# big-nacho/patolette

Hardware: AMD Instinct MI355X
Metric: Mpixels/sec quantized (256-color ICtCp + KMeans) at 1 GPU; palette ΔE vs ref (higher is better)
Workload: dtype f64

## Files before the change

include/patolette_amd.h:

```cpp
#ifndef PATOLETTE_AMD_H
#define PATOLETTE_AMD_H

#include <stddef.h>
#include <stdint.h>

#include "patolette.h"

#ifdef __cplusplus
extern "C" {
#endif

int  patolette_amd_device_count(void);
int  patolette_amd_set_device(int ordinal);
const char *patolette_amd_last_error(void);
void *patolette_amd_malloc(size_t bytes);
void patolette_amd_free(void *dptr);
int  patolette_amd_memcpy_h2d(void *dst, const void *src, size_t bytes);
int  patolette_amd_memcpy_d2h(void *dst, const void *src, size_t bytes);
int  patolette_amd_synchronize(void);
void patolette_amd_release_workspace(void);
int  patolette_amd_fill_image(double *d_planar, size_t n, uint64_t seed);
int  patolette_amd_fill_weights(double *d_weights, size_t n, uint64_t seed);

void patolette_amd_device(size_t width, size_t height, const double *d_data, const double *d_weights,
// ... 169 lines not shown
    PAMD_SRGB_TO_CIELUV = 1,
    PAMD_ICTCP_TO_REC2020 = 2,
    PAMD_CIELUV_TO_REC2020 = 3,
    PAMD_SRGB_TO_REC2020 = 4,
    PAMD_REC2020_TO_SRGB = 5,
    PAMD_CIELUV_TO_ICTCP = 6
};
int patolette_amd_convert(int which, double *planar, size_t n);

int patolette_amd_quantize_clusters(const double *colors, const double *weights, size_t n, size_t K,
                                    double *centers, size_t *n_clusters);

int patolette_amd_kmeans_refine(const double *colors, const double *weights, size_t n,
                                double *centers_io, size_t k, int niter, size_t max_samples);
int patolette_amd_debug_km_route(void);

int patolette_amd_nn_map(const double *colors, size_t n, const double *palette, size_t k, size_t *map);
int patolette_amd_debug_nn_route(int route);
int patolette_amd_debug_nn_map_elem(const double *colors, size_t n, const double *palette, size_t k, int map_elem_bytes, int misalign,
                                    void *map);

int patolette_amd_dither(const double *colors, size_t width, size_t height, const double *palette,
                         size_t k, size_t *map);

void patolette_amd_dither_config(int segments, int warm);
void patolette_amd_dither_layout(int lanes);
int patolette_amd_debug_dither_solo_cap(int cap);
int patolette_amd_debug_dither_stall_passes(int n);
int patolette_amd_dither_layout_in_use(size_t width, size_t height, size_t palette_rows);
void patolette_amd_debug_dither_locate(size_t width, size_t height, unsigned long long t, unsigned long long *d, unsigned long long *c);
// ... 54 lines not shown
```

patolette_amd/_native.py:

```python
import ctypes as C
import os

HERE = os.path.dirname(os.path.abspath(__file__))
LIB_PATH = os.path.join(HERE, "lib", "libpatolette_amd.so")

dp = C.POINTER(C.c_double)
zp = C.POINTER(C.c_size_t)


class QuantizationOptions(C.Structure):
    _fields_ = [("dither", C.c_bool), ("palette_only", C.c_bool), ("color_space", C.c_int),
                ("kmeans_niter", C.c_int), ("kmeans_max_samples", C.c_size_t), ("verbose", C.c_bool)]


class Stats(C.Structure):
    _fields_ = [(n, C.c_double) for n in ("ms_total", "ms_upload", "ms_convert", "ms_gq", "ms_lq",
                                          "ms_kmeans", "ms_map", "ms_download", "ms_saliency")] + \
               [(n, C.c_size_t) for n in ("n_base_clusters", "n_clusters", "split_evals", "split_px",
                                          "lq_rounds", "kmeans_samples", "dither_segments", "dither_repairs",
                                          "dither_rounds", "dither_through", "dither_jumps", "dither_solo")]

    def as_dict(self):
        return {n: getattr(self, n) for n, _ in self._fields_}

# ... 99 lines not shown
    "patolette_amd_hist_palette": (None, [C.c_void_p, C.c_int, C.c_size_t, C.POINTER(QuantizationOptions), dp, C.c_void_p,
                                          C.POINTER(C.c_int)]),
    "patolette_amd_batch": (None, [C.c_size_t, C.c_size_t, C.c_size_t, C.POINTER(dp), C.POINTER(dp), C.c_double, C.c_size_t,
                                   C.POINTER(QuantizationOptions), C.POINTER(dp), C.POINTER(zp), C.POINTER(C.c_int)]),
    "patolette_amd_batch_rows": (None, [C.c_size_t, C.c_size_t, C.c_size_t, C.POINTER(dp), C.POINTER(dp), C.c_double, C.c_size_t,
                                        C.POINTER(QuantizationOptions), C.POINTER(dp), C.POINTER(zp), C.POINTER(C.c_int)]),
    "patolette_amd_batch_u8": (None, [C.c_size_t, C.c_size_t, C.c_size_t, C.POINTER(C.c_void_p), C.c_int, C.POINTER(dp), C.c_double, C.c_size_t,
                                      C.POINTER(QuantizationOptions), C.POINTER(dp), C.POINTER(C.c_void_p), C.POINTER(C.c_void_p), C.c_int,
                                      C.POINTER(C.c_void_p), C.POINTER(C.c_int)]),
    "patolette_amd_pow": (C.c_int, [dp, C.c_double, dp, C.c_size_t]),
    "patolette_amd_convert": (C.c_int, [C.c_int, dp, C.c_size_t]),
    "patolette_amd_quantize_clusters": (C.c_int, [dp, dp, C.c_size_t, C.c_size_t, dp, zp]),
    "patolette_amd_kmeans_refine": (C.c_int, [dp, dp, C.c_size_t, dp, C.c_size_t, C.c_int, C.c_size_t]),
    "patolette_amd_nn_map": (C.c_int, [dp, C.c_size_t, dp, C.c_size_t, zp]),
    "patolette_amd_debug_km_route": (C.c_int, []),
    "patolette_amd_debug_nn_route": (C.c_int, [C.c_int]),
    "patolette_amd_debug_nn_map_elem": (C.c_int, [dp, C.c_size_t, dp, C.c_size_t, C.c_int, C.c_int, C.c_void_p]),
    "patolette_amd_set_global_quantiser": (C.c_int, [C.c_int]),
    "patolette_amd_dither": (C.c_int, [dp, C.c_size_t, C.c_size_t, dp, C.c_size_t, zp]),
    "patolette_amd_dither_config": (None, [C.c_int, C.c_int]),
    "patolette_amd_dither_layout": (None, [C.c_int]),
    "patolette_amd_debug_dither_solo_cap": (C.c_int, [C.c_int]),
    "patolette_amd_debug_dither_stall_passes": (C.c_int, [C.c_int]),
    "patolette_amd_dither_layout_in_use": (C.c_int, [C.c_size_t, C.c_size_t, C.c_size_t]),
    "patolette_amd_debug_dither_locate": (None, [C.c_size_t, C.c_size_t, C.c_ulonglong, C.POINTER(C.c_ulonglong),
                                                 C.POINTER(C.c_ulonglong)]),
    "patolette_amd_last_stats": (None, [C.POINTER(Stats)]),
    "patolette_amd_last_map_palette": (C.c_size_t, [dp, C.c_size_t]),
    "patolette_amd_last_split_trace": (C.c_size_t, [C.POINTER(SplitTrace), C.POINTER(SplitRecord), C.c_size_t]),
    "patolette_amd_last_cluster_centers": (C.c_size_t, [dp, C.c_size_t]),
# ... 79 lines not shown
```

patolette_amd/csrc/kmeans.h:

```cpp
#pragma once

#include "common.h"
#include "devutil.h"

namespace pamd {

constexpr int kKMeansMaxK = 4096;

struct KmSamples { float *x, *y, *z, *w; };

struct KMeansWork {
    DevBuf<float> sx, sy, sz, sw;
    DevBuf<int> assign;
    DevBuf<float4> sorted;
    DevBuf<unsigned int> table, rowtot, ticket;
    DevBuf<unsigned int> flags;
    DevBuf<unsigned int> rowbase;
    DevBuf<float> hs;
    DevBuf<float> cent, hassign;
    DevBuf<float4> c4;
    DevBuf<int> perm;
    DevBuf<struct DevMT> mt;
    bool mt_seeded = false;
    DevBuf<unsigned char> lut, grid, clist;
    DevBuf<unsigned int> mid;
    DevBuf<unsigned int> bkeys;
    DevBuf<unsigned long long> fsum;
    int route = 0;
    void reserve(size_t nx, int k);
};

enum KmRoute {
    KM_ROUTE_LIST = 1 << 0, KM_ROUTE_SCAN = 1 << 1, KM_ROUTE_BIGK = 1 << 2, KM_ROUTE_G32 = 1 << 3, KM_ROUTE_G64 = 1 << 4,
    KM_ROUTE_MID = 1 << 5, KM_ROUTE_SCATTER_INT = 1 << 6, KM_ROUTE_SCATTER_BYTE = 1 << 7, KM_ROUTE_SCATTER_PAIR = 1 << 8,
    KM_ROUTE_SCATTER_LDS = 1 << 9, KM_ROUTE_COOP = 1 << 10, KM_ROUTE_SUMS = 1 << 11
};

void kmeans_gather(const double *d_planar, size_t N, bool weighted, const int *d_perm, size_t nx, KMeansWork &w, hipStream_t s);
void kmeans_gather_slice(const double *d_planar, size_t n_local, bool weighted, const int *d_perm, size_t nx, size_t begin,
                         KMeansWork &w, hipStream_t s);
struct KmSums { double bound_x, bound_w; };
void kmeans_iterate(KMeansWork &w, size_t nx, int k, bool weighted, int niter, hipStream_t s, size_t expect_longest = 0,
                    const KmSums *sums = nullptr);

}
```

patolette_amd/csrc/kmeans.hip:

```cpp
#include "kmeans.h"

namespace pamd {

typedef __attribute__((address_space(1))) const void gvoid_t;
typedef __attribute__((address_space(3))) void lvoid_t;

template <bool W>
__global__ __launch_bounds__(256) void k_km_gather(const double *__restrict__ planar, size_t N, const int *__restrict__ perm,
                                                   size_t nx, KmSamples s) {
    const size_t stride = (size_t)gridDim.x * blockDim.x;
    for (size_t i = (size_t)blockIdx.x * blockDim.x + threadIdx.x; i < nx; i += stride) {
        size_t p = perm ? (size_t)perm[i] : i;
        s.x[i] = (float)planar[p]; s.y[i] = (float)planar[N + p]; s.z[i] = (float)planar[2 * N + p];
        if constexpr (W) s.w[i] = (float)planar[3 * N + p];
    }
}

template <bool W>
__global__ __launch_bounds__(256) void k_km_gather_slice(const double *__restrict__ planar, size_t n_local, const int *__restrict__ perm,
                                                         size_t nx, size_t begin, KmSamples s) {
    const size_t stride = (size_t)gridDim.x * blockDim.x;
    for (size_t i = (size_t)blockIdx.x * blockDim.x + threadIdx.x; i < nx; i += stride) {
        const size_t g = perm ? (size_t)perm[i] : i;
        const bool mine = g >= begin && g - begin < n_local;
// ... 1799 lines not shown
        __shared__ float s_hs[kKMeansMaxK];
        km_split_clusters_wave(cent, hassign, k, nx, mt, s_mt, s_hs, (int)threadIdx.x);
        __threadfence();
    }
    __syncthreads();
    for (int j = threadIdx.x; j < k; j += 256) km_store_c4(c4, k, j, cent[3 * j], cent[3 * j + 1], cent[3 * j + 2]);
}

static int chunk_len_for(size_t nx) {
    size_t c = ceil_div(nx, 4096);
    c = ceil_div(c, 64) * 64;
    if (c < 64) c = 64;
    return (int)c;
}

void KMeansWork::reserve(size_t nx, int k) {
    sx.reserve(nx); sy.reserve(nx); sz.reserve(nx); sw.reserve(nx);
    assign.reserve(nx); sorted.reserve(nx);
    const int nchunks = (int)ceil_div(nx, (size_t)chunk_len_for(nx));
    table.reserve(std::max((size_t)k * (size_t)(nchunks > 0 ? nchunks : 1),
                           (ceil_div(nx, (size_t)1024) * 257 + 1) / 2 + 1));
    rowtot.reserve(k);
    if (k > kKMeansMaxK) { rowbase.reserve(k); hs.reserve(k); }
    cent.reserve(3 * (size_t)k); hassign.reserve(k); c4.reserve(2 * (size_t)k + 2);
    perm.reserve(nx);
    if (!mt.p) { mt.reserve(1); mt_seeded = false; }
    if (!ticket.p) { ticket.reserve(1); HIP_CHECK(hipMemset(ticket.p, 0, sizeof(unsigned int))); }
    flags.reserve(2 + 256);
}

void kmeans_gather(const double *d_planar, size_t N, bool weighted, const int *d_perm, size_t nx, KMeansWork &w, hipStream_t s) {
    KmSamples ks{w.sx.p, w.sy.p, w.sz.p, w.sw.p};
    size_t g = ceil_div(nx, 256);
    if (g > 4096) g = 4096;
    if (g < 1) g = 1;
    KTIME("k_km_gather", s, (weighted ? 48.0 : 36.0) * nx);
// ... 2 lines not shown
    HIP_CHECK(hipGetLastError());
}

void kmeans_gather_slice(const double *d_planar, size_t n_local, bool weighted, const int *d_perm, size_t nx, size_t begin,
                         KMeansWork &w, hipStream_t s) {
    KmSamples ks{w.sx.p, w.sy.p, w.sz.p, w.sw.p};
    size_t g = ceil_div(nx, 256);
    if (g > 4096) g = 4096;
    if (g < 1) g = 1;
    KTIME("k_km_gather", s, (weighted ? 48.0 : 36.0) * nx);
    if (weighted) hipLaunchKernelGGL(k_km_gather_slice<true>, (int)g, 256, 0, s, d_planar, n_local, d_perm, nx, begin, ks);
    else hipLaunchKernelGGL(k_km_gather_slice<false>, (int)g, 256, 0, s, d_planar, n_local, d_perm, nx, begin, ks);
    HIP_CHECK(hipGetLastError());
}

void kmeans_iterate(KMeansWork &w, size_t nx, int k, bool weighted, int niter, hipStream_t s, size_t expect_longest, const KmSums *sums) {
    KmSamples ks{w.sx.p, w.sy.p, w.sz.p, w.sw.p};
    KmFix fix{};
    int ablocks = 1;
    if (sums && k > kKMeansMaxK) sums = nullptr;
    if (sums) {
        int ex = 0, ew = 0, P = 1;
        (void)frexp(std::max(sums->bound_x, 1e-300) * (weighted ? std::max(sums->bound_w, 1e-300) : 1.0), &ex);
        (void)frexp(std::max(sums->bound_w, 1e-300), &ew);
        while (((size_t)1 << P) < nx) P++;
        P = std::max(P + 1, 12);
        fix.quantum_x = ldexp(1.0, ex + P - 62); fix.magic_x = ldexp(1.5, 52 + ex + P - 62);
        fix.quantum_w = ldexp(1.0, ew + P - 62); fix.magic_w = ldexp(1.5, 52 + ew + P - 62);
        w.fsum.reserve(4 * (size_t)k);
        HIP_CHECK(hipMemsetAsync(w.fsum.p, 0, 4 * (size_t)k * sizeof(unsigned long long), s));
        ablocks = (int)std::min<size_t>(std::max<size_t>(ceil_div(nx, (size_t)4096), 1), 2048);
// ... 29 lines not shown
    const bool bigk = k > kKMeansMaxK;
    const size_t lds_cnt = bigk ? 0 : (size_t)8 * k * sizeof(unsigned int);
    const size_t lds_sct = (size_t)5 * k * sizeof(unsigned int);
    const size_t lds_sct_pair = (size_t)9 * k * sizeof(unsigned int) + (size_t)4 * (k + 64) * sizeof(float4);
    static PerDeviceOnce attr;
    attr.once([&] {
        HIP_CHECK(hipFuncSetAttribute((const void *)k_km_assign_count<false>, hipFuncAttributeMaxDynamicSharedMemorySize, 8 * kKMeansMaxK * 4));
        HIP_CHECK(hipFuncSetAttribute((const void *)k_km_scatter<true, int>, hipFuncAttributeMaxDynamicSharedMemorySize, 5 * kKMeansMaxK * 4));
        HIP_CHECK(hipFuncSetAttribute((const void *)k_km_scatter<false, int>, hipFuncAttributeMaxDynamicSharedMemorySize, 5 * kKMeansMaxK * 4));
        HIP_CHECK(hipFuncSetAttribute((const void *)k_km_scatter<true, unsigned char>, hipFuncAttributeMaxDynamicSharedMemorySize, 5 * kKMeansMaxK * 4));
        HIP_CHECK(hipFuncSetAttribute((const void *)k_km_scatter<false, unsigned char>, hipFuncAttributeMaxDynamicSharedMemorySize, 5 * kKMeansMaxK * 4));
        HIP_CHECK(hipFuncSetAttribute((const void *)k_km_update<true, false>, hipFuncAttributeMaxDynamicSharedMemorySize, 4 * 4096 * 4));
        HIP_CHECK(hipFuncSetAttribute((const void *)k_km_update<false, false>, hipFuncAttributeMaxDynamicSharedMemorySize, 4 * 4096 * 4));
    });
    if (!w.mt_seeded) { hipLaunchKernelGGL(k_km_mt_seed, 1, 1, 0, s, w.mt.p); w.mt_seeded = true; }
    { KTIME("k_km_prep", s, 28.0 * k); hipLaunchKernelGGL(k_km_prep, (std::max(k, kKmFlagWords) + 255) / 256, 256, 0, s, w.cent.p, k, w.c4.p, w.flags.p); }
    const size_t lut_min = getenv("PAMD_KM_LUT_MIN") ? (size_t)atoll(getenv("PAMD_KM_LUT_MIN")) : ((size_t)1 << 21);
    const bool use_lut = nx >= lut_min && k >= 16 && k <= 256;
    const size_t g64_min = getenv("PAMD_KM_G64_MIN") ? (size_t)atoll(getenv("PAMD_KM_G64_MIN")) : ((size_t)1 << 23);
    const int G = nx >= g64_min ? 64 : 32;
    if (use_lut) {
        static PerDeviceOnce attr2;
        attr2.once([&] {
            HIP_CHECK(hipFuncSetAttribute((const void *)k_km_assign_lut, hipFuncAttributeMaxDynamicSharedMemorySize, 8 * kKMeansMaxK * 4));
        });
        w.lut.reserve((size_t)G * G * G * 16); w.bkeys.reserve(kKmSlots * 6); w.grid.reserve(64 + sizeof(double));
        w.clist.reserve((size_t)(G * G * G / 64) * (2 + kKmCoarseMax));
        hipLaunchKernelGGL(k_km_bounds_init, 1, 256, 0, s, w.bkeys.p);
        { KTIME("k_km_bounds", s, 12.0 * nx); hipLaunchKernelGGL(k_km_bounds, (int)std::min<size_t>(ceil_div(nx, 256), 2048), 256, 0, s, ks, nx, w.bkeys.p); }
        hipLaunchKernelGGL(k_km_bounds_fold, 1, 64, 0, s, w.bkeys.p, (KmGridDev *)w.grid.p);
    }
    constexpr size_t direct_max = (size_t)1 << 19;
    const size_t list_longest = getenv("PAMD_KM_LIST_LONGEST") ? (size_t)atoll(getenv("PAMD_KM_LIST_LONGEST")) : (size_t)16384;
    const bool use_direct = !sums && !use_lut && k <= 256 && nx <= direct_max && nx < ((size_t)1 << 32) && expect_longest < list_longest;
    if (use_direct) {
        HIP_CHECK(hipMemsetAsync(w.assign.p, 0, nx, s));
        static PerDeviceOnce attr4;
        attr4.once([&] {
            HIP_CHECK(hipFuncSetAttribute((const void *)k_km_update_lists<true>, hipFuncAttributeMaxDynamicSharedMemorySize, kKmDirectCap * 20));
            HIP_CHECK(hipFuncSetAttribute((const void *)k_km_update_lists<false>, hipFuncAttributeMaxDynamicSharedMemorySize, kKmDirectCap * 20));
        });
    }
    const bool use_mid = use_lut && G == 64 && k % 8 == 0;
    if (use_mid) w.mid.reserve(32 * 32 * 32);
    const unsigned long long long_min = getenv("PAMD_KM_LONG_MIN") ? (unsigned long long)atoll(getenv("PAMD_KM_LONG_MIN")) : 8192ULL;
    int route = 0;
    for (int it = 0; it < niter; it++) {
        if (use_direct) {
            route |= KM_ROUTE_LIST;
            unsigned short *offs = (unsigned short *)w.table.p;
            const int sblocks = (int)ceil_div(nx, (size_t)kKmSortBlock);
// ... 129 lines not shown
```

patolette_amd/csrc/map.h:

```cpp
#pragma once

#include "common.h"

namespace pamd {

struct NNWork {
    DevBuf<unsigned char> lut;
    DevBuf<unsigned long long> keys;
    DevBuf<unsigned char> clist;
    DevBuf<unsigned int> mid;
    DevBuf<double> dtab;
    DevBuf<unsigned int> dside;
    PinBuf<unsigned int> hrep;
    DevBuf<double> dsort;
    DevBuf<unsigned int> dpos;
    size_t order_w = 0, order_h = 0; int order_dev = -1;
    DevBuf<unsigned int> dmpos;
    DevBuf<unsigned int> dmcnt;
    DevBuf<unsigned char> dsmap;
    DevBuf<unsigned char> dflag;
    size_t dither_segments = 0, dither_repairs = 0, dither_rounds = 0;
    size_t dither_through = 0;
    size_t dither_jumps = 0;
    size_t dither_solo = 0;
// ... 1 lines not shown
    hipEvent_t ev_fork = nullptr, ev_join = nullptr, ev_join2 = nullptr;
    int side_dev = -1;
    NNWork() = default;
    NNWork(const NNWork &) = delete;
    NNWork &operator=(const NNWork &) = delete;
    ~NNWork() {
        if (ev_fork) (void)hipEventDestroy(ev_fork);
        if (ev_join) (void)hipEventDestroy(ev_join);
        if (ev_join2) (void)hipEventDestroy(ev_join2);
        if (side_stream) (void)hipStreamDestroy(side_stream);
        if (side_stream2) (void)hipStreamDestroy(side_stream2);
    }
};
void launch_nn_map(const double *d_colors, size_t plane_stride, size_t n, const double *d_pal, int k,
                   void *d_out, int elem_bytes, const double *lo, const double *hi, NNWork &w, hipStream_t s);
int nn_debug_route(int route);
bool nn_map_u8_applies(size_t n, int k);
void launch_nn_map_u8(const unsigned char *d_px, int channels, size_t n, const double *d_pal, int k, void *d_out, int elem_bytes, NNWork &w, hipStream_t s);
bool dither_lane_layout(size_t width, size_t height, int k);
void launch_dither(const double *d_img, size_t plane_stride, int which, size_t width, size_t height, const double *d_pal, const double *h_pal, int k,
                   void *d_out, int elem_bytes, NNWork &w, hipStream_t s, int layout = -1);

constexpr size_t kDitherFramesMaxPixels = (size_t)1 << 31;
bool dither_frames_lane_layout(size_t frames, size_t width, size_t height, int k);
void launch_dither_frames(const double *d_img, size_t plane_stride, int which, size_t frames, size_t width, size_t height, const double *d_pal,
                          const double *h_pal, int k, void *d_out, int elem_bytes, NNWork &w, hipStream_t s, int layout = -1);

bool launch_dither_u8(const unsigned char *d_px, int channels, size_t frames, size_t width, size_t height, const double *d_pal, const double *h_pal,
                      int k, void *d_out, int elem_bytes, NNWork &w, hipStream_t s);

// ... 12 lines not shown
```

patolette_amd/csrc/map.hip:

```cpp
#include "map.h"
#include "compact.h"
#include "dither_slots.h"

#include <algorithm>
#include <atomic>
#include <cmath>
#include <mutex>
#include <type_traits>

#define PAMD_POW_TABLES_IN_LDS
#include "color_device.h"
#include "devutil.h"

namespace pamd {

template <typename OutT>
__global__ __launch_bounds__(256) void k_nn_map(const double *__restrict__ c, size_t N, size_t n, const double *__restrict__ pal, int k,
                                                OutT *__restrict__ out) {
    const double *palx = pal, *paly = pal + k, *palz = pal + 2 * k;
    const size_t stride = (size_t)gridDim.x * blockDim.x;
    for (size_t i = (size_t)blockIdx.x * blockDim.x + threadIdx.x; i < n; i += stride) {
        const double x = c[i], y = c[N + i], z = c[2 * N + i];
        double bd = INFINITY; int best = 0;
        for (int j = 0; j < k; j++) {
// ... 791 lines not shown
    attr_mid.once([&] { HIP_CHECK(hipFuncSetAttribute((const void *)(k_nn_map_mid<OutT, P, WAVES, NNSrcU8>), hipFuncAttributeMaxDynamicSharedMemorySize, (int)lds)); });
    const int blocks = (int)std::min<size_t>((size_t)num_cus(), ceil_div(n, (size_t)64 * WAVES * P));
    KTIME("k_nn_map_u8", s, ((double)channels + sizeof(OutT)) * n);
    hipLaunchKernelGGL((k_nn_map_mid<OutT, P, WAVES, NNSrcU8>), blocks, 64 * WAVES, lds, s, NNSrcU8{d_px, (size_t)channels}, n, d_pal, k, g, (const unsigned int *)w.mid.p,
                       (const float4 *)(w.mid.p + ncell / 8), (const unsigned char *)l1, (const unsigned char *)l2, out);
}
void launch_nn_map_u8(const unsigned char *d_px, int channels, size_t n, const double *d_pal, int k, void *d_out, int elem_bytes, NNWork &w, hipStream_t s) {
    if (!nn_map_u8_applies(n, k)) throw HipError("patolette_amd: the byte-source map kernel takes 2^22 .. 2^32 pixels and 8 .. 256 palette rows");
    if (channels != 3 && channels != 4) throw HipError("patolette_amd: 8-bit pixels have 3 or 4 channels");
    if (elem_bytes == 1) launch_nn_mid_u8<unsigned char>(d_px, channels, n, d_pal, k, (unsigned char *)d_out, w, s);
    else if (elem_bytes == 4) launch_nn_mid_u8<unsigned int>(d_px, channels, n, d_pal, k, (unsigned int *)d_out, w, s);
    else throw HipError("patolette_amd: the byte-source map kernel writes 1- or 4-byte elements");
    HIP_CHECK(hipGetLastError());
}

void launch_nn_map(const double *d_colors, size_t plane_stride, size_t n, const double *d_pal, int k, void *d_out, int elem_bytes,
                   const double *lo, const double *hi, NNWork &w, hipStream_t s) {
    if (elem_bytes != 1 && elem_bytes != 4 && elem_bytes != 8) throw HipError("patolette_amd: map element size must be 1, 4 or 8");
    const int cls = nn_size_class(n);
    bool use_lut = cls >= 1 && k >= 8 && k <= 4096;
    double blo[3] = {0, 0, 0}, bhi[3] = {0, 0, 0};
    if (use_lut) {
        if (lo && hi) { for (int a = 0; a < 3; a++) { blo[a] = lo[a]; bhi[a] = hi[a]; } }
        else {
            w.keys.reserve(6);
            unsigned long long init[6] = {~0ULL, ~0ULL, ~0ULL, 0ULL, 0ULL, 0ULL}, got[6];
            HIP_CHECK(hipMemcpyAsync(w.keys.p, init, sizeof init, hipMemcpyHostToDevice, s));
            { KTIME("k_minmax3", s, 24.0 * n); hipLaunchKernelGGL(k_minmax3, stream_blocks(n, 16), 256, 0, s, d_colors, plane_stride, n, w.keys.p); }
            HIP_CHECK(hipMemcpyAsync(got, w.keys.p, sizeof got, hipMemcpyDeviceToHost, s));
            HIP_CHECK(hipStreamSynchronize(s));
// ... 1652 lines not shown
```

patolette_amd/csrc/pipeline.hip:

```cpp
#include <algorithm>
#include <functional>
#include <chrono>
#include <cmath>
#include <atomic>
#include <memory>
#include <mutex>
#include <thread>
#include <future>
#include <type_traits>

#include "color_device.h"
#include "common.h"
#include "host_math.h"
#include "kmeans.h"
#include "map.h"
#include "ordered.h"
#include "delta.h"
#include "measure.h"
#include "lzw.h"
#include "hist.h"
#include "saliency.h"
#include "quant.h"
#include "rgba.h"
#include "compact.h"
// ... 866 lines not shown
    SalWork sal;
    DevBuf<double> wsal;
    DevBuf<GqDpDev> gq;
    PinBuf<GqDpDev> h_gq;
    DevBuf<GqOut> gqout;
    PinBuf<GqOut> h_gqout;
    PinBuf<double> h_pal;
    DevBuf<LqCtl> lqctl;
    PinBuf<LqHead> h_lqhead;
    PinBuf<LqRec> h_lqrec;
    PinBuf<LqCen> h_lqcen;
    std::vector<LqRec> lq_rec_local;
    std::vector<LqCommit> lq_commits;
    bool trace_pending = false;
    size_t lq_hint_N = 0, lq_hint_K = 0; int lq_hint_rounds = 0;
    DevBuf<int> perm_dev;
    size_t perm_N = 0, perm_nx = 0;
    PinBuf<int32_t> h_perm;
    size_t hperm_N = 0, hperm_nx = 0;
    hm::PermScratch perm_ws;
    std::future<void> perm_job;
    patolette_amd__Stats stats{};
    double ms_saliency = 0.0;
    std::string last_error;
    std::vector<double> map_palette;
    patolette_amd__SplitTrace trace_hdr{};
    std::vector<patolette_amd__SplitRecord> trace;
    std::vector<double> cluster_centers;

    void init() {
// ... 325 lines not shown
        }
        launch_hist(qlq, false, E.tilesA.p, ntA_ub, 0, E.nodes.p, E.hist.p, E.hsize.p, E.hcount.p, s, !rev, false, dyn, px_src);
        launch_cut(weighted, E.nodes.p, d_round, kLqRoundCap, E.hist.p, E.hsize.p, E.hcount.p, E.lut.p, s, dyn, nr_src);
        launch_partition(qlq, E.tilesP.p, ntP_ub, 0, d_round, d_tP0, kLqRoundCap, E.nodes.p, E.lut.p, E.tilecnt.p, E.tileoff.p, true, s, inv_sums, rev, dyn, px_src);
        enq++;
        control();
    };
    control();
    int want = (E.lq_hint_N == N && E.lq_hint_K == K && E.lq_hint_rounds > 0) ? E.lq_hint_rounds : 9;
    const bool fault_full = g_debug_fault.load(std::memory_order_relaxed) == 4;
    if (fault_full) want = 3;
    for (;;) {
        while (enq < want) round();
        hipLaunchKernelGGL(k_lq_export, 16, 256, 0, s, (const LqCtl *)c, head, E.h_lqrec.p, E.h_lqcen.p);
        HIP_CHECK(hipGetLastError());
        E.sync();
        if (fault_full) return -2;
        if (head->done) break;
        want = enq + 2;
    }
    if (head->error == 2) return -2;
    if (head->error == 3) return -1;
    if (kbase < 0) kbase = E.h_gqout.p->kbase;
    E.lq_hint_N = N; E.lq_hint_K = K; E.lq_hint_rounds = head->rounds;
    LqReplay rp;
    const double t_rp0 = now_ms();
    E.lq_rec_local.resize((size_t)head->nnodes);
    std::memcpy(E.lq_rec_local.data(), E.h_lqrec.p, (size_t)head->nnodes * sizeof(LqRec));
    const int fault = g_debug_fault.load(std::memory_order_relaxed);
    const bool replay_ok = lq_replay(E.lq_rec_local.data(), kbase, first_base, K, kDelta, fault, rp);
    const double t_rp1 = now_ms();
// ... 580 lines not shown
    return v < 0 ? env : v != 0;
}
static bool km_domain_ok(const double bound_x, const double bound_c, const bool weighted, const double bound_w, const double min_w, const size_t nx) {
    const double fmax = 3.4028234663852886e38, fmin = 1.1754943508222875e-38;
    const double B = std::max(1.0, std::max(bound_x, bound_c)), m = (double)std::min<size_t>(nx, (size_t)1 << 25);
    if (!(B < fmax) || !(bound_w < fmax)) return false;
    double Cb = 8.0 * B;
    if (weighted) {
        if (min_w > 0 && min_w < fmin) return false;
        const double by_n = std::exp(std::min((double)nx * 0x1p-23, 700.0)) * B;
        Cb = 4.0 * (min_w > 0 ? std::min(by_n, 4.0 * m * (std::max(bound_w, min_w) / min_w) * B) : by_n);
    }
    Cb += 8.0;
    return 16.0 * Cb * Cb <= fmax && 4.0 * m * std::max(bound_w, 1.0) * B <= fmax;
}
static void kmeans_refine(Engine &E, size_t N, bool weighted, std::vector<double> &centers, size_t k, int niter, size_t max_samples,
                          bool nonfinite, unsigned long long largest_cluster, double bound_x, double bound_w, double min_w = 0, bool bad_w = false) {
    hipStream_t s = E.stream;
    E.km.route = 0;
    const KmSums sums_v{bound_x, bound_w};
    const KmSums *sums = km_update_order_free() ? &sums_v : nullptr;
    std::vector<float> cent(3 * k);
    for (size_t i = 0; i < k; i++) for (int j = 0; j < 3; j++) cent[3 * i + j] = (float)centers[(size_t)j * k + i];
    const size_t min_samples = 256 * 256;
    const size_t ms = std::max(max_samples, min_samples);
    const int mppc = (int)(ms / k);
    const Shard *sh = E.shard;
    const size_t Nt = sh ? sh->total : N;
    auto expect_longest = [&](size_t nx_) { return (size_t)((double)largest_cluster / (double)(Nt ? Nt : 1) * (double)nx_); };
    bool ok = Nt >= k && !nonfinite && !bad_w;
    size_t nx = Nt;
    E.stats.kmeans_samples = 0;
    const bool sub = ok && Nt > k * (size_t)mppc;
    if (sub) nx = k * (size_t)mppc;
    if (ok && sub && nx < k + 1) ok = false;
    if (ok && nx != k) {
        double bound_c = 0;
        for (size_t i = 0; i < 3 * k; i++) bound_c = std::max(bound_c, std::fabs((double)cent[i]));
        for (size_t i = 0; i < 3 * k && ok; i++) ok = std::isfinite(cent[i]);
        ok = ok && km_domain_ok(bound_x, bound_c, weighted, bound_w, min_w, nx);
    }
    if (ok) {
        E.km.reserve(nx, (int)k);
        const int *dperm = nullptr;
        if (sub) dperm = subsample_list(E, Nt, nx, s);
        if (sh) {
            kmeans_gather_slice(E.cvt.p, N, weighted, dperm, nx, sh->begin, E.km, s);
            comm_sum_dev(E, E.km.sx.p, nx, 2); comm_sum_dev(E, E.km.sy.p, nx, 2); comm_sum_dev(E, E.km.sz.p, nx, 2);
            if (weighted) comm_sum_dev(E, E.km.sw.p, nx, 2);
            if (nx == k) {
                std::vector<float> f(3 * k);
                HIP_CHECK(hipMemcpy(f.data(), E.km.sx.p, k * sizeof(float), hipMemcpyDeviceToHost));
                HIP_CHECK(hipMemcpy(f.data() + k, E.km.sy.p, k * sizeof(float), hipMemcpyDeviceToHost));
                HIP_CHECK(hipMemcpy(f.data() + 2 * k, E.km.sz.p, k * sizeof(float), hipMemcpyDeviceToHost));
                for (size_t i = 0; i < k; i++) for (int j = 0; j < 3; j++) cent[3 * i + j] = f[(size_t)j * k + i];
            } else {
                HIP_CHECK(hipMemcpyAsync(E.km.cent.p, cent.data(), 3 * k * sizeof(float), hipMemcpyHostToDevice, s));
                HIP_CHECK(hipStreamSynchronize(s));
                kmeans_iterate(E.km, nx, (int)k, weighted, niter, s, expect_longest(nx), sums);
                HIP_CHECK(hipMemcpyAsync(cent.data(), E.km.cent.p, 3 * k * sizeof(float), hipMemcpyDeviceToHost, s));
                E.sync();
                E.stats.kmeans_samples = nx;
            }
        } else if (nx == k) {
            std::vector<double> first(3 * k);
            for (int j = 0; j < 3; j++) HIP_CHECK(hipMemcpy(first.data() + (size_t)j * k, E.cvt.p + (size_t)j * N, k * sizeof(double), hipMemcpyDeviceToHost));
            for (size_t i = 0; i < k; i++) for (int j = 0; j < 3; j++) cent[3 * i + j] = (float)first[(size_t)j * k + i];
        } else {
            kmeans_gather(E.cvt.p, N, weighted, dperm, nx, E.km, s);
            E.h_cent.reserve(3 * k);
            std::memcpy(E.h_cent.p, cent.data(), 3 * k * sizeof(float));
            HIP_CHECK(hipMemcpyAsync(E.km.cent.p, E.h_cent.p, 3 * k * sizeof(float), hipMemcpyHostToDevice, s));
            kmeans_iterate(E.km, nx, (int)k, weighted, niter, s, expect_longest(nx), sums);
            HIP_CHECK(hipMemcpyAsync(E.h_cent.p, E.km.cent.p, 3 * k * sizeof(float), hipMemcpyDeviceToHost, s));
            E.sync();
            std::memcpy(cent.data(), E.h_cent.p, 3 * k * sizeof(float));
            E.stats.kmeans_samples = nx;
        }
    }
    for (size_t i = 0; i < k; i++) for (int j = 0; j < 3; j++) centers[(size_t)j * k + i] = (double)cent[3 * i + j];
}

static void palette_rows(std::vector<double> &pal, size_t len, void (*f)(double[3])) {
    for (size_t i = 0; i < len; i++) {
        double c[3] = {pal[i], pal[len + i], pal[2 * len + i]};
        f(c);
        pal[i] = c[0]; pal[len + i] = c[1]; pal[2 * len + i] = c[2];
    }
}

// ... 86 lines not shown
static void copy_dither_stats(Engine &E) {
    E.stats.dither_segments = E.nn.dither_segments; E.stats.dither_repairs = E.nn.dither_repairs; E.stats.dither_rounds = E.nn.dither_rounds;
    E.stats.dither_through = E.nn.dither_through; E.stats.dither_jumps = E.nn.dither_jumps; E.stats.dither_solo = E.nn.dither_solo;
}
static bool map_touched(bool dither, size_t width, size_t height) { return !(dither && std::max(width, height) <= 1); }

static void run_device(Engine &E, size_t width, size_t height, Pixels px, const double *d_weights, size_t K,
                       const patolette__QuantizationOptions *opt, double *palette, void *d_map, int map_elem, const DitherMask *mask = nullptr,
                       const Frames *frames = nullptr) {
    hipStream_t s = E.stream;
    const size_t N = width * height;
    const bool weighted = d_weights != nullptr;
    const double t_start = now_ms();
    WsGuard wg(&E.stream, &E.stream2);
    E.stats = patolette_amd__Stats{};
    E.prep_N = 0;
    ws_prepare(E, N, K, weighted, opt->verbose);
    if (opt->kmeans_niter > 0) subsample_start(E, E.shard ? E.shard->total : N, K, opt->kmeans_max_samples);
    double t0 = now_ms();
    E.cvt.reserve((weighted ? 4 : 3) * N);
    E.cstats.reserve(1);
    if (E.shard && opt->dither && !opt->palette_only)
        throw HipError("patolette_amd: dithering walks the whole image along one curve; it is not available per slice");
    const ConvertPlan cp = convert_plan(E, opt, N);
    const int which = cp.which;
    const BinK sumk = cp.sumk, momk = cp.momk;
    if (px.converted) {  }
    else if (px.u8) launch_convert_u8(which, px.u8, px.channels, E.cvt.p, N, E.cstats.p, s, sumk, momk);
    else if (px.rows) launch_convert_rows(which, px.f64, E.cvt.p, N, E.cstats.p, s, sumk, momk);
    else launch_convert(which, px.f64, E.cvt.p, N, E.cstats.p, s, sumk, momk);
    if (weighted) {
        HIP_CHECK(hipMemcpyAsync(E.cvt.p + 3 * N, d_weights, N * sizeof(double), hipMemcpyDeviceToDevice, s));
        launch_weight_stats(d_weights, N, E.cstats.p, s);
    }
    Bounds bnd = read_bounds(E, weighted, [&] { gq_prepare(E, N, weighted); });
    bnd.have_sum = sumk.M0 != 0.0;
    bnd.have_mom = momk.M0 != 0.0;
    E.stats.ms_convert = now_ms() - t0;

    if (opt->verbose) printf("patolette ======== Palette generation \n");
    std::vector<double> pal;
    size_t len = 0;
    unsigned long long largest_cluster = 0;
    if (quantize_clusters(E, N, K, weighted, bnd, pal, len, opt->verbose, &largest_cluster) != 0) throw HipError("internal quantization error");

    t0 = now_ms();
    if (opt->kmeans_niter > 0) {
        if (opt->verbose) printf("patolette ======== KMeans refinement\n");
        kmeans_refine(E, N, weighted, pal, len, opt->kmeans_niter, opt->kmeans_max_samples, bnd.nonfinite, largest_cluster, bnd.cmax, bnd.wmax, bnd.wmin, bnd.bad_w);
    }
    E.stats.ms_kmeans = now_ms() - t0;

    t0 = now_ms();
    if (!opt->palette_only) {
        E.dpal.reserve(3 * len);
        if (opt->verbose) printf(opt->dither ? "patolette ======== Dithering\n" : "patolette ======== NN mapping\n");
        if (opt->dither) {
            int pix = PAMD_SRGB_TO_REC2020;
            void (*pf)(double[3]) = hm::color::srgb_to_rec2020;
            if (opt->color_space == patolette__CIELuv) { pix = PAMD_CIELUV_TO_REC2020; pf = hm::color::cieluv_to_rec2020; }
            else if (opt->color_space == patolette__ICtCp) { pix = PAMD_ICTCP_TO_REC2020; pf = hm::color::ictcp_to_rec2020; }
            palette_rows(pal, len, pf);
            E.map_palette = pal;
            if (d_map) {
                HIP_CHECK(hipMemcpyAsync(E.dpal.p, pal.data(), 3 * len * sizeof(double), hipMemcpyHostToDevice, s));
// ... 21 lines not shown
            const double *blo = bnd.lo, *bhi = bnd.hi;
            Bounds b2;
            if (opt->color_space == patolette__CIELuv) {
                if (d_map) {
                    E.aux.reserve(3 * N);
                    launch_convert(PAMD_CIELUV_TO_ICTCP, E.cvt.p, E.aux.p, N, E.cstats.p, s);
                    b2 = read_bounds(E, false);
                    blo = b2.lo; bhi = b2.hi;
                    pixels = E.aux.p;
                }
                palette_rows(pal, len, hm::color::cieluv_to_rec2020);
                palette_rows(pal, len, hm::color::rec2020_to_srgb);
                palette_rows(pal, len, hm::color::srgb_to_ictcp);
            }
            E.map_palette = pal;
            if (d_map) {
                E.h_pal.reserve(3 * len);
                upload_palette(E, pal, len);
                launch_nn_map(pixels, N, N, E.dpal.p, (int)len, d_map, map_elem, blo, bhi, E.nn, s);
            }
            palette_rows(pal, len, hm::color::ictcp_to_rec2020);
            palette_rows(pal, len, hm::color::rec2020_to_srgb);
        }
        E.sync();
    }
    E.stats.ms_map = now_ms() - t0;
    for (size_t j = 0; j < K * 3; j++) palette[j] = -1.0;
    for (int j = 0; j < 3; j++) for (size_t i = 0; i < len; i++) palette[K * (size_t)j + i] = pal[(size_t)j * len + i];
    E.stats.ms_total = now_ms() - t_start;
}

// ... 1742 lines not shown
        for (size_t i = 0; i < 3 * n && !nonfinite; i++) { nonfinite = !(std::fabs(colors[i]) < 0x1.ffffffp127); bx = std::max(bx, std::fabs(colors[i])); }
        bool bad_w = false;
        if (!nonfinite && weighted) for (size_t i = 0; i < n; i++) {
            const float wf = (float)weights[i];
            bw = std::max(bw, std::fabs(weights[i]));
            if (!(wf >= 0.f) || !std::isfinite(wf)) bad_w = true;
            else if (wf > 0.f && (min_w == 0 || (double)wf < min_w)) min_w = (double)wf;
        }
        kmeans_refine(E, n, weighted, pal, k, niter, max_samples, nonfinite, 0, bx, bw, min_w, bad_w);
        std::memcpy(centers_io, pal.data(), 3 * k * sizeof(double));
        return 0;
    });
}

int patolette_amd_debug_km_route(void) { return holder().e ? holder().e->km.route : 0; }

int patolette_amd_debug_nn_route(int route) { return nn_debug_route(route); }

int patolette_amd_debug_nn_map_elem(const double *colors, size_t n, const double *palette, size_t k, int map_elem_bytes, int misalign, void *map) {
    return guarded([&](Engine &E) -> int {
        const int eb = map_elem_bytes;
        if ((eb != 1 && eb != 4 && eb != 8) || (eb == 1 && k > 256) || k == 0 || (misalign != 0 && (misalign != 1 || eb != 1)))
            throw HipError("patolette_amd_debug_nn_map_elem: elements of 1 (up to 256 rows), 4 or 8 bytes; misalign 0, or 1 with 1-byte elements");
        if (n == 0) return 0;
        E.src.reserve(3 * n); E.dpal.reserve(3 * k); E.dmap.reserve(n * (size_t)eb + 1);
        HIP_CHECK(hipMemcpy(E.src.p, colors, 3 * n * sizeof(double), hipMemcpyHostToDevice));
        HIP_CHECK(hipMemcpy(E.dpal.p, palette, 3 * k * sizeof(double), hipMemcpyHostToDevice));
        launch_nn_map(E.src.p, n, n, E.dpal.p, (int)k, E.dmap.p + misalign, eb, nullptr, nullptr, E.nn, E.stream);
        E.sync();
        HIP_CHECK(hipMemcpy(map, E.dmap.p + misalign, n * (size_t)eb, hipMemcpyDeviceToHost));
// ... 86 lines not shown
```

Measured before the change: 3122.

## Overlap KMeans sample gather with LQ export and enqueue NN map after KMeans

While the host waits on the local-quantizer export, the KMeans subsample gather and setup are now queued on the device ahead of time. After KMeans refinement, the centers are written to the device palette in f64 and the nearest-neighbour map is launched before the host sync. This removes host-device round trips between pipeline stages. In exchange it needs capacity-fit checks, event-based syncs and more complex fallback logic, and if the predicted sample count differs from the actual one it forces an extra sync.

```diff
diff --git a/include/patolette_amd.h b/include/patolette_amd.h
--- a/include/patolette_amd.h
+++ b/include/patolette_amd.h
@@ -207,6 +207,7 @@
 int patolette_amd_kmeans_refine(const double *colors, const double *weights, size_t n,
                                 double *centers_io, size_t k, int niter, size_t max_samples);
 int patolette_amd_debug_km_route(void);
+int patolette_amd_debug_handoff(void);
 
 int patolette_amd_nn_map(const double *colors, size_t n, const double *palette, size_t k, size_t *map);
 int patolette_amd_debug_nn_route(int route);
diff --git a/patolette_amd/_native.py b/patolette_amd/_native.py
--- a/patolette_amd/_native.py
+++ b/patolette_amd/_native.py
@@ -137,6 +137,7 @@
     "patolette_amd_kmeans_refine": (C.c_int, [dp, dp, C.c_size_t, dp, C.c_size_t, C.c_int, C.c_size_t]),
     "patolette_amd_nn_map": (C.c_int, [dp, C.c_size_t, dp, C.c_size_t, zp]),
     "patolette_amd_debug_km_route": (C.c_int, []),
+    "patolette_amd_debug_handoff": (C.c_int, []),
     "patolette_amd_debug_nn_route": (C.c_int, [C.c_int]),
     "patolette_amd_debug_nn_map_elem": (C.c_int, [dp, C.c_size_t, dp, C.c_size_t, C.c_int, C.c_int, C.c_void_p]),
     "patolette_amd_set_global_quantiser": (C.c_int, [C.c_int]),
diff --git a/patolette_amd/csrc/kmeans.h b/patolette_amd/csrc/kmeans.h
--- a/patolette_amd/csrc/kmeans.h
+++ b/patolette_amd/csrc/kmeans.h
@@ -28,6 +28,7 @@
     DevBuf<unsigned long long> fsum;
     int route = 0;
     void reserve(size_t nx, int k);
+    bool fits(size_t nx, int k) const;
 };
 
 enum KmRoute {
@@ -41,6 +42,8 @@
                          KMeansWork &w, hipStream_t s);
 struct KmSums { double bound_x, bound_w; };
 void kmeans_iterate(KMeansWork &w, size_t nx, int k, bool weighted, int niter, hipStream_t s, size_t expect_longest = 0,
-                    const KmSums *sums = nullptr);
+                    const KmSums *sums = nullptr, bool setup_done = false);
+void kmeans_setup(KMeansWork &w, size_t nx, int k, hipStream_t s);
+void kmeans_export_palette(const KMeansWork &w, int k, double *d_pal, hipStream_t s);
 
 }
diff --git a/patolette_amd/csrc/kmeans.hip b/patolette_amd/csrc/kmeans.hip
--- a/patolette_amd/csrc/kmeans.hip
+++ b/patolette_amd/csrc/kmeans.hip
@@ -1837,12 +1837,23 @@
     return (int)c;
 }
 
+static size_t table_words_for(size_t nx, int k) {
+    const int nchunks = (int)ceil_div(nx, (size_t)chunk_len_for(nx));
+    return std::max((size_t)k * (size_t)(nchunks > 0 ? nchunks : 1),
+                    (ceil_div(nx, (size_t)1024) * 257 + 1) / 2 + 1);
+}
+
+bool KMeansWork::fits(size_t nx, int k) const {
+    const size_t uk = (size_t)k;
+    return sx.cap >= nx && sy.cap >= nx && sz.cap >= nx && sw.cap >= nx && assign.cap >= nx && sorted.cap >= nx &&
+           table.cap >= table_words_for(nx, k) && rowtot.cap >= uk && (k <= kKMeansMaxK || (rowbase.cap >= uk && hs.cap >= uk)) &&
+           cent.cap >= 3 * uk && hassign.cap >= uk && c4.cap >= 2 * uk + 2 && perm.cap >= nx && mt.p && ticket.p && flags.cap >= 2 + 256;
+}
+
 void KMeansWork::reserve(size_t nx, int k) {
     sx.reserve(nx); sy.reserve(nx); sz.reserve(nx); sw.reserve(nx);
     assign.reserve(nx); sorted.reserve(nx);
-    const int nchunks = (int)ceil_div(nx, (size_t)chunk_len_for(nx));
-    table.reserve(std::max((size_t)k * (size_t)(nchunks > 0 ? nchunks : 1),
-                           (ceil_div(nx, (size_t)1024) * 257 + 1) / 2 + 1));
+    table.reserve(table_words_for(nx, k));
     rowtot.reserve(k);
     if (k > kKMeansMaxK) { rowbase.reserve(k); hs.reserve(k); }
     cent.reserve(3 * (size_t)k); hassign.reserve(k); c4.reserve(2 * (size_t)k + 2);
@@ -1875,7 +1886,35 @@
     HIP_CHECK(hipGetLastError());
 }
 
-void kmeans_iterate(KMeansWork &w, size_t nx, int k, bool weighted, int niter, hipStream_t s, size_t expect_longest, const KmSums *sums) {
+static bool km_use_lut(size_t nx, int k) {
+    const size_t lut_min = getenv("PAMD_KM_LUT_MIN") ? (size_t)atoll(getenv("PAMD_KM_LUT_MIN")) : ((size_t)1 << 21);
+    return nx >= lut_min && k >= 16 && k <= 256;
+}
+static bool km_list_sizes(size_t nx, int k) {
+    constexpr size_t direct_max = (size_t)1 << 19;
+    return !km_use_lut(nx, k) && k <= 256 && nx <= direct_max && nx < ((size_t)1 << 32);
+}
+
+void kmeans_setup(KMeansWork &w, size_t nx, int k, hipStream_t s) {
+    if (!w.mt_seeded) { hipLaunchKernelGGL(k_km_mt_seed, 1, 1, 0, s, w.mt.p); w.mt_seeded = true; }
+    hipLaunchKernelGGL(k_km_prep, (kKmFlagWords + 255) / 256, 256, 0, s, (const float *)nullptr, 0, (float4 *)nullptr, w.flags.p);
+    if (km_list_sizes(nx, k)) HIP_CHECK(hipMemsetAsync(w.assign.p, 0, nx, s));
+    HIP_CHECK(hipGetLastError());
+}
+
+__global__ __launch_bounds__(256) void k_km_palette_f64(const float *__restrict__ cent, int k, double *__restrict__ pal) {
+    const int i = blockIdx.x * blockDim.x + threadIdx.x;
+    if (i >= k) return;
+#pragma unroll
+    for (int j = 0; j < 3; j++) pal[(size_t)j * k + i] = (double)cent[3 * i + j];
+}
+void kmeans_export_palette(const KMeansWork &w, int k, double *d_pal, hipStream_t s) {
+    hipLaunchKernelGGL(k_km_palette_f64, (k + 255) / 256, 256, 0, s, (const float *)w.cent.p, k, d_pal);
+    HIP_CHECK(hipGetLastError());
+}
+
+void kmeans_iterate(KMeansWork &w, size_t nx, int k, bool weighted, int niter, hipStream_t s, size_t expect_longest, const KmSums *sums,
+                    bool setup_done) {
     KmSamples ks{w.sx.p, w.sy.p, w.sz.p, w.sw.p};
     KmFix fix{};
     int ablocks = 1;
@@ -1935,9 +1974,12 @@
         HIP_CHECK(hipFuncSetAttribute((const void *)k_km_update<false, false>, hipFuncAttributeMaxDynamicSharedMemorySize, 4 * 4096 * 4));
     });
     if (!w.mt_seeded) { hipLaunchKernelGGL(k_km_mt_seed, 1, 1, 0, s, w.mt.p); w.mt_seeded = true; }
-    { KTIME("k_km_prep", s, 28.0 * k); hipLaunchKernelGGL(k_km_prep, (std::max(k, kKmFlagWords) + 255) / 256, 256, 0, s, w.cent.p, k, w.c4.p, w.flags.p); }
-    const size_t lut_min = getenv("PAMD_KM_LUT_MIN") ? (size_t)atoll(getenv("PAMD_KM_LUT_MIN")) : ((size_t)1 << 21);
-    const bool use_lut = nx >= lut_min && k >= 16 && k <= 256;
+    {
+        KTIME("k_km_prep", s, 28.0 * k);
+        hipLaunchKernelGGL(k_km_prep, ((setup_done ? k : std::max(k, kKmFlagWords)) + 255) / 256, 256, 0, s, w.cent.p, k, w.c4.p,
+                           setup_done ? (unsigned int *)nullptr : w.flags.p);
+    }
+    const bool use_lut = km_use_lut(nx, k);
     const size_t g64_min = getenv("PAMD_KM_G64_MIN") ? (size_t)atoll(getenv("PAMD_KM_G64_MIN")) : ((size_t)1 << 23);
     const int G = nx >= g64_min ? 64 : 32;
     if (use_lut) {
@@ -1951,11 +1993,10 @@
         { KTIME("k_km_bounds", s, 12.0 * nx); hipLaunchKernelGGL(k_km_bounds, (int)std::min<size_t>(ceil_div(nx, 256), 2048), 256, 0, s, ks, nx, w.bkeys.p); }
         hipLaunchKernelGGL(k_km_bounds_fold, 1, 64, 0, s, w.bkeys.p, (KmGridDev *)w.grid.p);
     }
-    constexpr size_t direct_max = (size_t)1 << 19;
     const size_t list_longest = getenv("PAMD_KM_LIST_LONGEST") ? (size_t)atoll(getenv("PAMD_KM_LIST_LONGEST")) : (size_t)16384;
-    const bool use_direct = !sums && !use_lut && k <= 256 && nx <= direct_max && nx < ((size_t)1 << 32) && expect_longest < list_longest;
+    const bool use_direct = !sums && km_list_sizes(nx, k) && expect_longest < list_longest;
     if (use_direct) {
-        HIP_CHECK(hipMemsetAsync(w.assign.p, 0, nx, s));
+        if (!setup_done) HIP_CHECK(hipMemsetAsync(w.assign.p, 0, nx, s));
         static PerDeviceOnce attr4;
         attr4.once([&] {
             HIP_CHECK(hipFuncSetAttribute((const void *)k_km_update_lists<true>, hipFuncAttributeMaxDynamicSharedMemorySize, kKmDirectCap * 20));
diff --git a/patolette_amd/csrc/map.h b/patolette_amd/csrc/map.h
--- a/patolette_amd/csrc/map.h
+++ b/patolette_amd/csrc/map.h
@@ -39,6 +39,7 @@
 };
 void launch_nn_map(const double *d_colors, size_t plane_stride, size_t n, const double *d_pal, int k,
                    void *d_out, int elem_bytes, const double *lo, const double *hi, NNWork &w, hipStream_t s);
+bool nn_map_fits(const NNWork &w, size_t n, int k);
 int nn_debug_route(int route);
 bool nn_map_u8_applies(size_t n, int k);
 void launch_nn_map_u8(const unsigned char *d_px, int channels, size_t n, const double *d_pal, int k, void *d_out, int elem_bytes, NNWork &w, hipStream_t s);
diff --git a/patolette_amd/csrc/map.hip b/patolette_amd/csrc/map.hip
--- a/patolette_amd/csrc/map.hip
+++ b/patolette_amd/csrc/map.hip
@@ -829,6 +829,16 @@
     HIP_CHECK(hipGetLastError());
 }
 
+bool nn_map_fits(const NNWork &w, size_t n, int k) {
+    const int cls = nn_size_class(n);
+    if (!(cls >= 1 && k >= 8 && k <= 4096)) return true;
+    const int G = cls == 2 ? 64 : 32;
+    const size_t ncell = (size_t)G * G * G, ncoarse = ncell / 64;
+    if (w.clist.cap < ncoarse * (1 + kCoarseMax) * 2) return false;
+    if (k > 256) return w.lut.cap >= ncell * 64;
+    return w.lut.cap >= ncell * 32 && (G != 64 || w.mid.cap >= ncell / 8 + 257 * 4);
+}
+
 void launch_nn_map(const double *d_colors, size_t plane_stride, size_t n, const double *d_pal, int k, void *d_out, int elem_bytes,
                    const double *lo, const double *hi, NNWork &w, hipStream_t s) {
     if (elem_bytes != 1 && elem_bytes != 4 && elem_bytes != 8) throw HipError("patolette_amd: map element size must be 1, 4 or 8");
diff --git a/patolette_amd/csrc/pipeline.hip b/patolette_amd/csrc/pipeline.hip
--- a/patolette_amd/csrc/pipeline.hip
+++ b/patolette_amd/csrc/pipeline.hip
@@ -904,6 +904,8 @@
     std::vector<LqCommit> lq_commits;
     bool trace_pending = false;
     size_t lq_hint_N = 0, lq_hint_K = 0; int lq_hint_rounds = 0;
+    const std::function<void()> *lq_behind_export = nullptr;
+    int handoff = 0;
     DevBuf<int> perm_dev;
     size_t perm_N = 0, perm_nx = 0;
     PinBuf<int32_t> h_perm;
@@ -1259,7 +1261,12 @@
         while (enq < want) round();
         hipLaunchKernelGGL(k_lq_export, 16, 256, 0, s, (const LqCtl *)c, head, E.h_lqrec.p, E.h_lqcen.p);
         HIP_CHECK(hipGetLastError());
-        E.sync();
+        if (E.lq_behind_export) {
+            if (!E.ev_stats) HIP_CHECK(hipEventCreateWithFlags(&E.ev_stats, hipEventDisableTiming));
+            HIP_CHECK(hipEventRecord(E.ev_stats, s));
+            (*E.lq_behind_export)();
+            HIP_CHECK(hipEventSynchronize(E.ev_stats));
+        } else E.sync();
         if (fault_full) return -2;
         if (head->done) break;
         want = enq + 2;
@@ -1870,8 +1877,15 @@
     Cb += 8.0;
     return 16.0 * Cb * Cb <= fmax && 4.0 * m * std::max(bound_w, 1.0) * B <= fmax;
 }
+struct KmHandoff {
+    bool early_done = false; size_t early_nx = 0, early_k = 0;
+    double *dpal = nullptr; const std::function<void()> *then = nullptr;
+    bool early_used = false, handed = false;
+};
+
 static void kmeans_refine(Engine &E, size_t N, bool weighted, std::vector<double> &centers, size_t k, int niter, size_t max_samples,
-                          bool nonfinite, unsigned long long largest_cluster, double bound_x, double bound_w, double min_w = 0, bool bad_w = false) {
+                          bool nonfinite, unsigned long long largest_cluster, double bound_x, double bound_w, double min_w = 0, bool bad_w = false,
+                          KmHandoff *ho = nullptr) {
     hipStream_t s = E.stream;
     E.km.route = 0;
     const KmSums sums_v{bound_x, bound_w};
@@ -1896,10 +1910,12 @@
         for (size_t i = 0; i < 3 * k && ok; i++) ok = std::isfinite(cent[i]);
         ok = ok && km_domain_ok(bound_x, bound_c, weighted, bound_w, min_w, nx);
     }
+    const bool early = ho && ho->early_done && ok && !sh && nx != k && ho->early_nx == nx && ho->early_k == k;
+    if (ho && ho->early_done && !early) E.sync();
     if (ok) {
         E.km.reserve(nx, (int)k);
         const int *dperm = nullptr;
-        if (sub) dperm = subsample_list(E, Nt, nx, s);
+        if (sub && !early) dperm = subsample_list(E, Nt, nx, s);
         if (sh) {
             kmeans_gather_slice(E.cvt.p, N, weighted, dperm, nx, sh->begin, E.km, s);
             comm_sum_dev(E, E.km.sx.p, nx, 2); comm_sum_dev(E, E.km.sy.p, nx, 2); comm_sum_dev(E, E.km.sz.p, nx, 2);
@@ -1923,13 +1939,22 @@
             for (int j = 0; j < 3; j++) HIP_CHECK(hipMemcpy(first.data() + (size_t)j * k, E.cvt.p + (size_t)j * N, k * sizeof(double), hipMemcpyDeviceToHost));
             for (size_t i = 0; i < k; i++) for (int j = 0; j < 3; j++) cent[3 * i + j] = (float)first[(size_t)j * k + i];
         } else {
-            kmeans_gather(E.cvt.p, N, weighted, dperm, nx, E.km, s);
+            if (!early) kmeans_gather(E.cvt.p, N, weighted, dperm, nx, E.km, s);
             E.h_cent.reserve(3 * k);
             std::memcpy(E.h_cent.p, cent.data(), 3 * k * sizeof(float));
             HIP_CHECK(hipMemcpyAsync(E.km.cent.p, E.h_cent.p, 3 * k * sizeof(float), hipMemcpyHostToDevice, s));
-            kmeans_iterate(E.km, nx, (int)k, weighted, niter, s, expect_longest(nx), sums);
+            kmeans_iterate(E.km, nx, (int)k, weighted, niter, s, expect_longest(nx), sums, early);
+            if (ho) ho->early_used = early;
+            const bool hand = ho && ho->dpal && ho->then;
+            if (hand) kmeans_export_palette(E.km, (int)k, ho->dpal, s);
             HIP_CHECK(hipMemcpyAsync(E.h_cent.p, E.km.cent.p, 3 * k * sizeof(float), hipMemcpyDeviceToHost, s));
-            E.sync();
+            if (hand) {
+                if (!E.ev_stats) HIP_CHECK(hipEventCreateWithFlags(&E.ev_stats, hipEventDisableTiming));
+                HIP_CHECK(hipEventRecord(E.ev_stats, s));
+                (*ho->then)();
+                ho->handed = true;
+                HIP_CHECK(hipEventSynchronize(E.ev_stats));
+            } else E.sync();
             std::memcpy(cent.data(), E.h_cent.p, 3 * k * sizeof(float));
             E.stats.kmeans_samples = nx;
         }
@@ -2046,6 +2071,7 @@
     const double t_start = now_ms();
     WsGuard wg(&E.stream, &E.stream2);
     E.stats = patolette_amd__Stats{};
+    E.handoff = 0;
     E.prep_N = 0;
     ws_prepare(E, N, K, weighted, opt->verbose);
     if (opt->kmeans_niter > 0) subsample_start(E, E.shard ? E.shard->total : N, K, opt->kmeans_max_samples);
@@ -2074,13 +2100,44 @@
     std::vector<double> pal;
     size_t len = 0;
     unsigned long long largest_cluster = 0;
-    if (quantize_clusters(E, N, K, weighted, bnd, pal, len, opt->verbose, &largest_cluster) != 0) throw HipError("internal quantization error");
+    KmHandoff ho;
+    if (opt->kmeans_niter > 0 && !E.shard && K > 0 && N >= K && !bnd.nonfinite && !bnd.bad_w) {
+        const size_t ms = std::max(opt->kmeans_max_samples, (size_t)(256 * 256));
+        const size_t nxK = K * (size_t)(int)(ms / K);
+        const bool sub = N > nxK;
+        const size_t nx = sub ? nxK : N;
+        const bool list_fits = !sub || (E.perm_N == N && E.perm_nx >= nx) || (E.hperm_N == N && E.hperm_nx >= nx && E.perm_dev.cap >= E.hperm_nx);
+        if (nx != K && nx >= K + 1 && list_fits && E.km.fits(nx, (int)K)) { ho.early_nx = nx; ho.early_k = K; }
+    }
+    const std::function<void()> early = [&] {
+        if (ho.early_done || !ho.early_k) return;
+        const int *dperm = N > ho.early_nx ? subsample_list(E, N, ho.early_nx, s) : nullptr;
+        kmeans_gather(E.cvt.p, N, weighted, dperm, ho.early_nx, E.km, s);
+        kmeans_setup(E.km, ho.early_nx, (int)ho.early_k, s);
+        ho.early_done = true;
+    };
+    struct BehindExport {
+        Engine &E;
+        BehindExport(Engine &e, const std::function<void()> *f) : E(e) { E.lq_behind_export = f; }
+        ~BehindExport() { E.lq_behind_export = nullptr; }
+    };
+    {
+        BehindExport be(E, &early);
+        if (quantize_clusters(E, N, K, weighted, bnd, pal, len, opt->verbose, &largest_cluster) != 0) throw HipError("internal quantization error");
+    }
 
     t0 = now_ms();
+    const std::function<void()> map_behind = [&] { launch_nn_map(E.cvt.p, N, N, E.dpal.p, (int)len, d_map, map_elem, bnd.lo, bnd.hi, E.nn, s); };
+    if (opt->kmeans_niter > 0 && !opt->palette_only && !opt->dither && d_map && !E.shard && opt->color_space != patolette__CIELuv &&
+        E.dpal.cap >= 3 * len && nn_map_fits(E.nn, N, (int)len)) {
+        ho.dpal = E.dpal.p; ho.then = &map_behind;
+    }
     if (opt->kmeans_niter > 0) {
         if (opt->verbose) printf("patolette ======== KMeans refinement\n");
-        kmeans_refine(E, N, weighted, pal, len, opt->kmeans_niter, opt->kmeans_max_samples, bnd.nonfinite, largest_cluster, bnd.cmax, bnd.wmax, bnd.wmin, bnd.bad_w);
-    }
+        kmeans_refine(E, N, weighted, pal, len, opt->kmeans_niter, opt->kmeans_max_samples, bnd.nonfinite, largest_cluster, bnd.cmax, bnd.wmax, bnd.wmin,
+                      bnd.bad_w, &ho);
+    }
+    E.handoff = (ho.early_used ? 1 : 0) | (ho.early_done && !ho.early_used ? 2 : 0) | (ho.handed ? 4 : 0);
     E.stats.ms_kmeans = now_ms() - t0;
 
     t0 = now_ms();
@@ -2132,7 +2189,7 @@
                 palette_rows(pal, len, hm::color::srgb_to_ictcp);
             }
             E.map_palette = pal;
-            if (d_map) {
+            if (d_map && !ho.handed) {
                 E.h_pal.reserve(3 * len);
                 upload_palette(E, pal, len);
                 launch_nn_map(pixels, N, N, E.dpal.p, (int)len, d_map, map_elem, blo, bhi, E.nn, s);
@@ -3905,6 +3962,7 @@
 }
 
 int patolette_amd_debug_km_route(void) { return holder().e ? holder().e->km.route : 0; }
+int patolette_amd_debug_handoff(void) { return holder().e ? holder().e->handoff : 0; }
 
 int patolette_amd_debug_nn_route(int route) { return nn_debug_route(route); }
 
```

Result: no change. 3145 (median of 6 runs) (+0.7%).
